# chenghuige/golden-huffman

Measured on AMD Instinct MI355X. Metric: encode+decode GB/s (input bytes), higher is better.
Workload: dtype u8

## Files before the change

### golden-huffman_amd/csrc/ghf_api.hip

```cpp
#include <algorithm>
#include <cstdio>
#include <cstring>
#include <new>
#include <string>

#include "ghf_code_rules.h"
#include "ghf_ctx.h"

using namespace ghf;

namespace {

thread_local std::string g_create_err;

int ensure_ws(ghf_ctx* c, size_t nchunks) {
  bool new_off = false, new_hist = false;
  int rc = grow(c, c->chunk_off, nchunks + 1, 1024, &new_off);
  if (!rc) rc = grow(c, c->chunk_hist, nchunks * 256, 1024 * 256, &new_hist);
  if (new_off) c->plan.forget();
  if (new_hist) c->hist.forget();
  return rc;
}

}
// ... 178 lines not shown
}

const char* ghf_last_error(ghf_ctx* c) { return c ? c->err.c_str() : g_create_err.c_str(); }

int ghf_device_alloc(ghf_ctx* c, size_t bytes, void** d_ptr) {
  if (!c || !d_ptr) return GHF_E_INVAL;
  GHF_HIP(c, hipSetDevice(c->device));
  GHF_HIP(c, hipMalloc(d_ptr, bytes ? bytes : 16));
  return GHF_OK;
}
int ghf_device_free(ghf_ctx* c, void* d_ptr) {
  if (!c) return GHF_E_INVAL;
  if (d_ptr) {
    GHF_HIP(c, hipSetDevice(c->device));
    GHF_HIP(c, hipStreamSynchronize(c->stream));
    GHF_HIP(c, hipFree(d_ptr));
  }
  return GHF_OK;
}
int ghf_host_alloc(ghf_ctx* c, size_t bytes, void** h_ptr) {
  if (!c || !h_ptr) return GHF_E_INVAL;
  GHF_HIP(c, hipSetDevice(c->device));
  GHF_HIP(c, hipHostMalloc(h_ptr, bytes ? bytes : 16, hipHostMallocDefault));
  return GHF_OK;
}
int ghf_host_free(ghf_ctx* c, void* h_ptr) {
  if (!c) return GHF_E_INVAL;
  if (h_ptr) GHF_HIP(c, hipHostFree(h_ptr));
  return GHF_OK;
}
int ghf_copy_h2d(ghf_ctx* c, void* d_dst, const void* h_src, size_t bytes) {
  if (!c || (bytes && (!d_dst || !h_src))) return GHF_E_INVAL;
  GHF_HIP(c, hipSetDevice(c->device));
  if (bytes) GHF_HIP(c, hipMemcpyAsync(d_dst, h_src, bytes, hipMemcpyHostToDevice, c->stream));
  return GHF_OK;
}
int ghf_copy_d2h(ghf_ctx* c, void* h_dst, const void* d_src, size_t bytes) {
  if (!c || (bytes && (!h_dst || !d_src))) return GHF_E_INVAL;
  GHF_HIP(c, hipSetDevice(c->device));
  if (bytes) GHF_HIP(c, hipMemcpyAsync(h_dst, d_src, bytes, hipMemcpyDeviceToHost, c->stream));
  return GHF_OK;
}
int ghf_copy_d2d(ghf_ctx* c, void* d_dst, const void* d_src, size_t bytes, int non_temporal) {
  if (!c || (bytes && (!d_dst || !d_src))) return GHF_E_INVAL;
  if (!aligned16(d_dst) || !aligned16(d_src)) return fail(c, GHF_E_INVAL, "ghf_copy_d2d: 16-byte aligned pointers");
  GHF_HIP(c, hipSetDevice(c->device));
  if (bytes) launch_stream_copy(static_cast<const uint8_t*>(d_src), static_cast<uint8_t*>(d_dst), bytes, non_temporal != 0, c->stream);
  return GHF_OK;
}
int ghf_memset_d(ghf_ctx* c, void* d_dst, int value, size_t bytes) {
  if (!c || (bytes && !d_dst)) return GHF_E_INVAL;
  GHF_HIP(c, hipSetDevice(c->device));
  if (bytes) GHF_HIP(c, hipMemsetAsync(d_dst, value, bytes, c->stream));
  return GHF_OK;
}

struct ghf_event {
  int device = 0;
  hipEvent_t ev = nullptr;
};
int ghf_event_create(ghf_ctx* c, ghf_event** out) {
  if (!c || !out) return GHF_E_INVAL;
  GHF_HIP(c, hipSetDevice(c->device));
  ghf_event* e = new (std::nothrow) ghf_event;
  if (!e) return fail(c, GHF_E_HIP, "out of host memory");
  e->device = c->device;
  const hipError_t rc = hipEventCreateWithFlags(&e->ev, hipEventDisableTiming);
  if (rc != hipSuccess) {
    delete e;
    return fail(c, GHF_E_HIP, "hipEventCreateWithFlags", rc);
  }
  *out = e;
  return GHF_OK;
}
int ghf_event_destroy(ghf_event* e) {
  if (!e) return GHF_OK;
  (void)hipSetDevice(e->device);
  if (e->ev) (void)hipEventDestroy(e->ev);
  delete e;
  return GHF_OK;
}
int ghf_event_record(ghf_ctx* c, ghf_event* e) {
  if (!c || !e) return GHF_E_INVAL;
  GHF_HIP(c, hipSetDevice(c->device));
  GHF_HIP(c, hipEventRecord(e->ev, c->stream));
  return GHF_OK;
}
int ghf_event_wait(ghf_ctx* c, ghf_event* e) {
  if (!c || !e) return GHF_E_INVAL;
  GHF_HIP(c, hipSetDevice(c->device));
  GHF_HIP(c, hipStreamWaitEvent(c->stream, e->ev, 0));
  return GHF_OK;
}
int ghf_event_sync(ghf_event* e) {
  if (!e) return GHF_E_INVAL;
  if (hipSetDevice(e->device) != hipSuccess) return GHF_E_HIP;
  return hipEventSynchronize(e->ev) == hipSuccess ? GHF_OK : GHF_E_HIP;
}

uint32_t ghf_chunk_symbols(size_t n) { return chunk_symbols_for(n); }
size_t ghf_header_bytes(int max_len) { return header_bytes_for((size_t)max_len); }

size_t ghf_compress_bound(size_t n) {
  const size_t bits = 9 * (n + 1);
  size_t b = header_bytes_for(32) + (bits + 7) / 8;
  return ((b + 15) & ~(size_t)15) + 16;
}

static int histogram(ghf_ctx* c, const uint8_t* d_in, size_t n, uint64_t* d_hist, bool add) {
  if (!c || !d_hist || (n && !d_in)) return GHF_E_INVAL;
  GHF_HIP(c, hipSetDevice(c->device));
  const uint32_t cl = chunk_symbols_for(n);
  const size_t nchunks = (size_t)chunk_count_for(n);
  int rc = ensure_ws(c, nchunks);
  if (rc) return rc;
  launch_histogram(d_in, n, cl, (uint32_t)nchunks, c->chunk_hist.p, d_hist, c->d_hist_acc, add, c->stream);
  GHF_HIP(c, hipGetLastError());
  if (add) c->hist.forget();
  else c->hist = {d_in, n, cl};
  return GHF_OK;
}
int ghf_histogram(ghf_ctx* c, const uint8_t* d_in, size_t n, uint64_t* d_hist) { return histogram(c, d_in, n, d_hist, false); }
int ghf_histogram_add(ghf_ctx* c, const uint8_t* d_in, size_t n, uint64_t* d_hist) { return histogram(c, d_in, n, d_hist, true); }

int ghf_build_code_ex(ghf_ctx* c, const uint64_t* d_hist, ghf_code* d_code, unsigned flags) {
  if (!c || !d_hist || !d_code || (flags & ~(unsigned)(GHF_CODE_LIMIT | GHF_EMPTY_OK))) return GHF_E_INVAL;
  GHF_HIP(c, hipSetDevice(c->device));
  launch_build_code(d_hist, d_code, c->d_status, flags, c->stream);
  GHF_HIP(c, hipGetLastError());
  if (c->plan.code == d_code) c->plan.forget();
  if (c->prepared.describes(d_code)) c->prepared.forget();
  return GHF_OK;
}

int ghf_build_code(ghf_ctx* c, const uint64_t* d_hist, ghf_code* d_code) { return ghf_build_code_ex(c, d_hist, d_code, 0); }

int ghf_write_header(ghf_ctx* c, const ghf_code* d_code, uint8_t* d_out, size_t cap) {
  if (!c || !d_code || !d_out || (reinterpret_cast<uintptr_t>(d_out) & 3u)) return GHF_E_INVAL;
  GHF_HIP(c, hipSetDevice(c->device));
  launch_write_header(d_code, d_out, cap, c->d_status, c->stream);
  GHF_HIP(c, hipGetLastError());
  return GHF_OK;
}

int ghf_encode_plan(ghf_ctx* c, const uint8_t* d_in, size_t n, const ghf_code* d_code, uint64_t* d_total_bits) {
  if (!c || !d_code || (n && !d_in)) return GHF_E_INVAL;
  GHF_HIP(c, hipSetDevice(c->device));
  const uint32_t cl = chunk_symbols_for(n);
  const size_t nchunks = (size_t)chunk_count_for(n);
  int rc = ensure_ws(c, nchunks);
  if (rc) return rc;
  const bool have_hist = c->hist.describes(d_in, n, cl) && n != 0;
  launch_plan(d_in, n, cl, (uint32_t)nchunks, have_hist ? c->chunk_hist.p : nullptr, d_code, c->chunk_off.p,
              d_total_bits ? d_total_bits : &c->d->total_bits, c->stream);
  GHF_HIP(c, hipGetLastError());
  c->plan = {d_in, n, d_code};
  return GHF_OK;
}

int ghf_encode_emit(ghf_ctx* c, const uint8_t* d_in, size_t n, const ghf_code* d_code, const uint64_t* d_start_bit,
                    int flags, uint8_t* d_out, size_t cap, const ghf_index* index, uint64_t* d_end) {
  if (!c || !d_code || !d_out || (n && !d_in)) return GHF_E_INVAL;
  if (!aligned16(d_out)) return fail(c, GHF_E_INVAL, "d_out must be 16-byte aligned");
  if ((flags & GHF_EMIT_HEADER) && (flags & GHF_EMIT_REBASE))
    return fail(c, GHF_E_INVAL, "GHF_EMIT_HEADER is for the buffer that starts at stream byte 0 (rank 0 / single GPU)");
  if (!c->plan.describes(d_in, n, d_code))
    return fail(c, GHF_E_INVAL, "ghf_encode_emit: call ghf_encode_plan on the same (d_in, n, d_code) first");
  GHF_HIP(c, hipSetDevice(c->device));
  const uint32_t cl = chunk_symbols_for(n);
  const size_t nchunks = (size_t)chunk_count_for(n);
  if (index && (index->n_symbols != n || !index_has_arrays(index)))
    return fail(c, GHF_E_INVAL, "ghf_encode_emit: index does not match n (use ghf_index_alloc)");
  EmitParams p;
  p.in = d_in;
  p.n = n;
  p.code = d_code;
  p.chunk_off = c->chunk_off.p;
  p.d_start_bit = d_start_bit;
  p.out = d_out;
  p.cap = cap;
  p.chunk = cl;
  p.nchunks = (uint32_t)nchunks;
  p.chunk_bit = index ? index->d_chunk_bit : nullptr;
  p.seg_bit = index ? index->d_seg_bit : nullptr;
  p.flags = flags;
  p.status = c->d_status;
  p.d_end = d_end;
  launch_emit(p, c->stream);
  GHF_HIP(c, hipGetLastError());
  return GHF_OK;
}

int ghf_shard_start_bit(ghf_ctx* c, const ghf_code* d_code, const uint64_t* d_totals, int world, int rank,
                        uint64_t* d_start_bit) {
  if (!c || !d_code || !d_totals || !d_start_bit || world < 1 || rank < 0 || rank >= world) return GHF_E_INVAL;
  GHF_HIP(c, hipSetDevice(c->device));
  launch_shard_start(d_code, d_totals, rank, d_start_bit, c->stream);
  GHF_HIP(c, hipGetLastError());
  return GHF_OK;
}

int ghf_compress(ghf_ctx* c, const uint8_t* d_in, size_t n, uint8_t* d_out, size_t cap, uint64_t* d_out_bytes,
                 ghf_code* d_code, const ghf_index* index) {
  return ghf_compress_ex(c, d_in, n, d_out, cap, d_out_bytes, d_code, index, 0);
}

int ghf_compress_ex(ghf_ctx* c, const uint8_t* d_in, size_t n, uint8_t* d_out, size_t cap, uint64_t* d_out_bytes,
                    ghf_code* d_code, const ghf_index* index, unsigned code_flags) {
  if (!c || !d_out || (n && !d_in)) return GHF_E_INVAL;
  if (n == 0 && !(code_flags & GHF_EMPTY_OK)) return fail(c, GHF_E_EMPTY, "empty input is undefined in the reference; refused");
  if (!aligned16(d_out)) return fail(c, GHF_E_INVAL, "d_out must be 16-byte aligned");
  ghf_code* code = d_code ? d_code : c->d_code;
  int rc;
  if (n == 0) {
    const size_t hdr = ghf_header_bytes(1);
    if (cap < hdr + 1) return fail(c, GHF_E_CAP, "ghf_compress: capacity below the 1049 bytes of the empty stream");
    if ((rc = ghf_histogram(c, d_in, 0, c->d_hist))) return rc;
    if ((rc = ghf_build_code_ex(c, c->d_hist, code, code_flags))) return rc;
    if ((rc = ghf_write_header(c, code, d_out, cap))) return rc;
    GHF_HIP(c, hipMemsetAsync(d_out + hdr, 0x7F, 1, c->stream));
    if (d_out_bytes) {
      launch_store_u64(d_out_bytes, nullptr, hdr + 1, c->stream);
      GHF_HIP(c, hipGetLastError());
    }
    return GHF_OK;
  }
  if ((rc = ghf_histogram(c, d_in, n, c->d_hist))) return rc;
  if ((rc = ghf_build_code_ex(c, c->d_hist, code, code_flags))) return rc;
  if ((rc = ghf_encode_plan(c, d_in, n, code, &c->d->total_bits))) return rc;
  if ((rc = ghf_encode_emit(c, d_in, n, code, nullptr, GHF_EMIT_LAST | GHF_EMIT_HEADER, d_out, cap, index, c->d->end))) return rc;
  if (d_out_bytes) {
    launch_store_u64(d_out_bytes, &c->d->end[1], 0, c->stream);
    GHF_HIP(c, hipGetLastError());
  }
  return GHF_OK;
}

int ghf_index_alloc(ghf_ctx* c, size_t n_symbols, ghf_index* out) {
  if (!c || !out) return GHF_E_INVAL;
  GHF_HIP(c, hipSetDevice(c->device));
  std::memset(out, 0, sizeof *out);
  index_shape(n_symbols, out);
  GHF_HIP(c, hipMalloc(&out->d_chunk_bit, std::max<size_t>(out->n_chunks, 1) * sizeof(uint64_t)));
  hipError_t e = hipMalloc(&out->d_seg_bit, std::max<size_t>(out->n_segs, 1) * sizeof(uint32_t));
  if (e != hipSuccess) {
    (void)hipFree(out->d_chunk_bit);
    out->d_chunk_bit = nullptr;
    return fail(c, GHF_E_HIP, "hipMalloc(seg_bit)", e);
  }
  return GHF_OK;
}

int ghf_index_free(ghf_ctx* c, ghf_index* idx) { return free_index_arrays(c, idx); }

size_t ghf_compress_batch_bound(size_t max_item_bytes) { return ghf_compress_bound(max_item_bytes); }

int ghf_batch_index_alloc(ghf_ctx* c, uint32_t count, size_t max_item_bytes, ghf_batch_index* out) {
  if (!c || !out || max_item_bytes == 0 || max_item_bytes > GHF_BATCH_MAX_ITEM) return GHF_E_INVAL;
  GHF_HIP(c, hipSetDevice(c->device));
  std::memset(out, 0, sizeof *out);
  out->count = count;
  out->max_item_bytes = max_item_bytes;
  out->blocks_per_item = blocks_for(max_item_bytes);
  out->segs_per_item = segs_for(max_item_bytes);
  GHF_HIP(c, hipMalloc(&out->d_chunk_bit, std::max<size_t>((size_t)count * out->blocks_per_item, 1) * sizeof(uint64_t)));
  hipError_t e = hipMalloc(&out->d_seg_bit, std::max<size_t>((size_t)count * out->segs_per_item, 1) * sizeof(uint32_t));
  if (e != hipSuccess) {
    (void)hipFree(out->d_chunk_bit);
    out->d_chunk_bit = nullptr;
    return fail(c, GHF_E_HIP, "hipMalloc(batch seg_bit)", e);
  }
  return GHF_OK;
}

int ghf_batch_index_free(ghf_ctx* c, ghf_batch_index* idx) { return free_index_arrays(c, idx); }

int ghf_batch_index_item(const ghf_batch_index* idx, uint32_t i, size_t n_i, ghf_index* view) {
  if (!idx || !view || i >= idx->count || n_i > idx->max_item_bytes) return GHF_E_INVAL;
  std::memset(view, 0, sizeof *view);
  index_shape(n_i, view);
  view->d_chunk_bit = idx->d_chunk_bit ? idx->d_chunk_bit + (size_t)i * idx->blocks_per_item : nullptr;
  view->d_seg_bit = idx->d_seg_bit ? idx->d_seg_bit + (size_t)i * idx->segs_per_item : nullptr;
  return GHF_OK;
}

static bool batch_index_covers(const ghf_batch_index* ix, uint32_t count, size_t max_item_bytes) {
  return ix->d_chunk_bit && ix->d_seg_bit && ix->count >= count && ix->max_item_bytes >= max_item_bytes &&
         ix->max_item_bytes <= GHF_BATCH_MAX_ITEM &&
         ix->blocks_per_item == blocks_for(ix->max_item_bytes) && ix->segs_per_item == segs_for(ix->max_item_bytes);
}

int ghf_compress_batch(ghf_ctx* c, const uint8_t* const* d_in_ptrs, const uint64_t* d_in_bytes, size_t max_item_bytes,
                       uint32_t count, uint8_t* const* d_out_ptrs, const uint64_t* d_out_caps, uint64_t* d_out_bytes,
                       ghf_code* d_codes, const ghf_batch_index* index, int* d_item_status) {
  if (!c) return GHF_E_INVAL;
  if (max_item_bytes == 0 || max_item_bytes > GHF_BATCH_MAX_ITEM)
    return fail(c, GHF_E_INVAL, "ghf_compress_batch: max_item_bytes must be 1 .. GHF_BATCH_MAX_ITEM");
  if (index && !batch_index_covers(index, count, max_item_bytes))
    return fail(c, GHF_E_INVAL, "ghf_compress_batch: index does not cover (count, max_item_bytes) (use ghf_batch_index_alloc)");
  if (count == 0) return GHF_OK;
  if (!d_in_ptrs || !d_in_bytes || !d_out_ptrs || !d_out_caps || !d_out_bytes || !d_item_status) return GHF_E_INVAL;
  GHF_HIP(c, hipSetDevice(c->device));
  if (!d_codes) {
    const int rc = grow(c, c->batch_codes, count);
    if (rc) return rc;
    d_codes = c->batch_codes.p;
  }
// ... 1095 lines not shown
```

### golden-huffman_amd/csrc/ghf_internal.h

```cpp
#ifndef GHF_INTERNAL_H_
#define GHF_INTERNAL_H_
#include <hip/hip_runtime.h>
#include <stdint.h>
#include <type_traits>
#include "ghf.h"

namespace ghf {

constexpr int kWave = 64;
constexpr int kSymPerLane = 16;
constexpr int kSymPerIter = kWave * kSymPerLane;
constexpr int kSegSymbols = 64;
constexpr int kBlockSymbols = 4096;
constexpr uint32_t kChunkQuantum = 4096;
constexpr uint32_t kMinChunk = 16384;
constexpr uint32_t kMaxChunk = 1u << 20;
constexpr uint32_t kEmitSlots = 256 * 3 * 8;

constexpr int kHistThreads = 256;
constexpr int kHistRep = 32;

constexpr int kEmitThreads = 512;
constexpr int kEmitWaves = kEmitThreads / kWave;
constexpr int kStageWords = 544;
// ... 191 lines not shown
};

struct BatchHistParams {
  const uint8_t* const* in_ptrs;
  const uint64_t* in_bytes;
  uint64_t max_item_bytes;
  uint32_t count;
  uint64_t* hist;
};
struct BatchSharedCompressParams {
  const uint8_t* const* in_ptrs;
  const uint64_t* in_bytes;
  uint64_t max_item_bytes;
  const ghf_code* code;
  uint8_t* const* out_ptrs;
  const uint64_t* out_caps;
  uint64_t* out_bytes;
  uint64_t* chunk_bit;
  uint32_t* seg_bit;
  uint64_t blocks_per_item, segs_per_item;
  int* item_status;
};
struct BatchSharedDecodeParams {
  const uint8_t* const* stream_ptrs;
  const uint64_t* stream_bytes;
  const ghf_code* code;
  const uint64_t* chunk_bit;
  const uint32_t* seg_bit;
  uint64_t blocks_per_item, segs_per_item;
  uint64_t max_item_bytes;
  const uint64_t* n_symbols;
  uint8_t* const* out_ptrs;
  const uint64_t* out_caps;
  uint64_t* out_bytes;
  int* item_status;
};
struct BatchSharedBodiesParams {
  const uint8_t* const* stream_ptrs;
  const uint64_t* stream_bytes;
  uint64_t max_stream_bytes;
  const ghf_code* code;
  uint8_t* const* out_ptrs;
  const uint64_t* out_caps;
  uint64_t* out_bytes;
  int* item_status;
  uint64_t* stats;
};

struct BatchPlanesHistParams {
  const uint8_t* const* in_ptrs;
  const uint64_t* in_bytes;
  uint64_t max_item_bytes;
  uint32_t count;
  uint64_t* hists;
};
struct BatchPlanesCompressParams {
  const uint8_t* const* in_ptrs;
  const uint64_t* in_bytes;
  uint64_t max_item_bytes;
  const ghf_code* codes;
  uint8_t* const* out_ptrs;
  const uint64_t* out_caps;
  uint64_t* out_bytes;
  uint64_t* chunk_bit;
  uint32_t* seg_bit;
  uint64_t blocks_per_item, segs_per_item;
  int* item_status;
};
struct BatchPlanesDecodeParams {
  const uint8_t* const* stream_ptrs;
  const uint64_t* stream_bytes;
  const ghf_code* codes;
  const uint64_t* chunk_bit;
  const uint32_t* seg_bit;
  uint64_t blocks_per_item, segs_per_item;
  uint64_t max_plane_symbols;
  const uint64_t* n_elems;
  uint8_t* const* out_ptrs;
  const uint64_t* out_caps;
  uint64_t* out_bytes;
  int* item_status;
};
struct BatchPlanesBodiesParams {
  const uint8_t* const* stream_ptrs;
  const uint64_t* stream_bytes;
  uint64_t max_stream_bytes;
  const ghf_code* codes;
  uint8_t* const* out_ptrs;
  const uint64_t* out_caps;
  uint64_t* out_bytes;
  int* item_status;
  uint64_t* stats;
};

constexpr uint32_t kBatchSeekMagic = 0x31524247u;
constexpr uint32_t kBatchRunSymbols = 128;
constexpr uint32_t kBatchRunSegs = kBatchRunSymbols / kSegSymbols;
constexpr uint32_t kBatchRunsPerBlock = kBlockSymbols / kBatchRunSymbols;
constexpr uint32_t kBatchSeekHeadBytes = 8;
__host__ __device__ constexpr inline uint64_t batch_runs_for(uint64_t n) { return (n + kBatchRunSymbols - 1) / kBatchRunSymbols; }
__host__ __device__ constexpr inline uint64_t batch_seek_bytes_for(uint64_t n) {
  return (kBatchSeekHeadBytes + 2 * batch_runs_for(n) + 7) & ~7ull;
}
struct BatchSeekPackParams {
  const uint64_t* chunk_bit;
  const uint32_t* seg_bit;
  uint64_t blocks_per_item, segs_per_item;
  uint64_t max_slice_symbols;
  const uint64_t* in_bytes;
  uint32_t elem_bytes;
  uint8_t* const* rec_ptrs;
  const uint64_t* rec_caps;
  uint64_t* rec_bytes;
  int* slot_status;
};
struct BatchSeekDecodeParams {
  const uint8_t* const* stream_ptrs;
  const uint64_t* stream_bytes;
  const uint8_t* const* rec_ptrs;
  const uint64_t* rec_bytes;
  uint64_t max_stream_bytes;
  const ghf_code* codes;
  uint8_t* const* out_ptrs;
  const uint64_t* out_caps;
  uint64_t* out_bytes;
  int* item_status;
};

enum SyncKind : uint32_t {
  kSyncCrs2 = 0,
  kSyncCrs = 1,
  kSyncPiece = 2,
};
struct SyncParams {
  const uint8_t* stream;
  uint64_t stream_bytes;
  uint64_t body_bit0;
  uint64_t end_bit;
  uint32_t no_eof;
  const DecTables* dt;
  uint64_t nsub;
  uint16_t* start;
  uint16_t* used;
  uint32_t* cnt;
  uint8_t* eof;
  uint32_t first;
  uint32_t first_start;
  uint32_t* changed;
  unsigned long long* moved_first_inv;
  uint64_t* eof_sub;
  uint64_t* tile_sum;
};

constexpr size_t kHistAccWords = 32 * 256 + 16 + 16 * 16;
void launch_histogram(const uint8_t* d_in, uint64_t n, uint32_t chunk, uint32_t nchunks, uint32_t* d_chunk_hist,
                      uint64_t* d_hist, uint64_t* d_acc, bool add, hipStream_t s);
void launch_build_code(const uint64_t* d_hist, ghf_code* d_code, int* d_status, uint32_t flags, hipStream_t s);
void launch_write_header(const ghf_code* d_code, uint8_t* d_out, uint64_t cap, int* d_status, hipStream_t s);
void launch_plan(const uint8_t* d_in, uint64_t n, uint32_t chunk, uint32_t nchunks, const uint32_t* d_chunk_hist,
                 const ghf_code* d_code, uint64_t* d_chunk_off, uint64_t* d_total_bits, hipStream_t s);
void launch_scan(uint64_t* d_v, uint32_t count, uint64_t* d_total, hipStream_t s);
void launch_crs_build_code(const uint64_t* d_hist, ghf_tree* d_tree, ghf_code* d_code, uint64_t* d_start_bit, int* d_status,
                           hipStream_t s);
void launch_crs_finish(const ghf_tree* d_tree, const uint64_t* d_total_bits, uint8_t* d_out, uint64_t* d_out_bytes, int* d_status,
                       hipStream_t s);
void launch_stream_copy(const uint8_t* d_src, uint8_t* d_dst, uint64_t n, bool nt, hipStream_t s);
void launch_store_u64(uint64_t* d_dst, const uint64_t* d_src_opt, uint64_t add, hipStream_t s);
void launch_load_u16(uint64_t* d_dst, const uint16_t* d_src, hipStream_t s);
void launch_shard_start(const ghf_code* d_code, const uint64_t* d_totals, int rank, uint64_t* d_start_bit, hipStream_t s);
void launch_emit(const EmitParams& p, hipStream_t s);
void launch_build_decode_tables(const ghf_code* d_code, DecTables* d_dt, int* d_status, hipStream_t s);
void launch_build_decode_tables_slots(const ghf_code* d_codes, DecTables* d_dts, uint32_t count, uint32_t slots, int* d_status, hipStream_t s);
void launch_crs_decode_tables(const ghf_tree* d_tree, DecTables* d_dt, int* d_status, hipStream_t s);
constexpr uint64_t kDecMaxGroups = 0xFFFF0000ull;
void launch_decode(const DecParams& p, hipStream_t s);
void launch_sync_pass(const SyncParams& p, hipStream_t s);
void launch_sync_counts(const SyncParams& p, uint64_t* d_total, hipStream_t s);
size_t sync_scan_workspace(uint64_t nsub);
void launch_sync_scan(const SyncParams& p, uint8_t* ws, uint32_t stride ,
                      uint32_t entry , hipStream_t s);
void launch_sync_index(const SyncParams& p, uint64_t* d_seg_abs, uint64_t n_symbols, uint64_t* d_chunk_bit, uint32_t* d_seg_bit,
                       hipStream_t s);
void launch_seek_pack(const SeekPackParams& p, hipStream_t s);
void launch_seek_expand(const SeekExpandParams& p, hipStream_t s);
void launch_seek_expand_planes(const SeekExpandPlanesParams& a, uint32_t planes, hipStream_t s);
void launch_seek_expand_streams(const SeekExpandStreamsParams& a, uint32_t streams, hipStream_t s);
void launch_decode_head(const DecHeadParams& p, hipStream_t s);
void launch_compress_batch(const BatchCompressParams& p, uint32_t count, hipStream_t s);
void launch_decode_batch(const BatchDecodeParams& p, uint32_t count, hipStream_t s);
void launch_decode_images_batch(const BatchImagesParams& p, uint32_t count, hipStream_t s);
void launch_histogram_batch(const BatchHistParams& p, uint32_t flags, hipStream_t s);
void launch_compress_batch_shared(const BatchSharedCompressParams& p, uint32_t count, hipStream_t s);
void launch_decode_batch_shared(const BatchSharedDecodeParams& p, uint32_t count, hipStream_t s);
void launch_decode_bodies_batch_shared(const BatchSharedBodiesParams& p, uint32_t count, hipStream_t s);
void launch_histogram_batch_finish(uint64_t* d_hists, uint32_t n_hists, uint32_t flags, hipStream_t s);
void launch_histogram_batch_planes(const BatchPlanesHistParams& p, uint32_t elem_bytes, uint32_t flags, hipStream_t s);
void launch_build_codes(const uint64_t* d_hists, uint32_t n_codes, ghf_code* d_codes, int* d_status, uint32_t flags, hipStream_t s);
void launch_batch_planes_raw_auto(const uint64_t* d_hists, const ghf_code* d_codes, uint32_t elem_bytes, uint32_t* d_raw_planes,
                                  hipStream_t s);
void launch_compress_batch_planes(const BatchPlanesCompressParams& p, uint32_t count, uint32_t elem_bytes, bool forms, uint32_t raw_planes,
                                  hipStream_t s);
void launch_decode_batch_planes(const BatchPlanesDecodeParams& p, uint32_t count, uint32_t elem_bytes, bool forms, uint32_t raw_planes,
                                hipStream_t s);
void launch_decode_bodies_batch_planes(const BatchPlanesBodiesParams& p, uint32_t count, uint32_t elem_bytes, bool forms,
                                       uint32_t raw_planes, hipStream_t s);
void launch_batch_seek_pack(const BatchSeekPackParams& p, uint32_t slots, hipStream_t s);
void launch_decode_bodies_batch_seek(const BatchSeekDecodeParams& p, uint32_t count, uint32_t elem_bytes, bool forms, uint32_t raw_planes,
                                     hipStream_t s);
void launch_planes_split(const uint8_t* d_in, const uint8_t* d_base, uint64_t n_elems, uint32_t elem_bytes, uint8_t* d_planes,
                         uint64_t plane_stride, hipStream_t s);
void launch_planes_merge(const uint8_t* d_planes, uint64_t plane_stride, const uint8_t* d_base, uint64_t n_elems, uint32_t elem_bytes,
                         uint8_t* d_out, const int* d_status, hipStream_t s);
void launch_planes_merge_range(const uint8_t* d_planes, uint64_t plane_stride, const uint8_t* d_base, uint64_t first, uint64_t count,
                               uint32_t elem_bytes, uint8_t* d_out, const int* d_status, hipStream_t s);
void launch_planes_split_to(const uint8_t* d_in, const uint8_t* d_base, uint64_t n_elems, uint32_t elem_bytes, uint8_t* const* h_dst,
                            hipStream_t s);
void launch_planes_merge_from(const uint8_t* const* h_src, const uint8_t* d_base, uint64_t n_elems, uint32_t elem_bytes, uint8_t* d_out,
                              const int* d_status, hipStream_t s);
void launch_sparse_split(const uint8_t* d_in, uint64_t n, uint8_t* d_mask, uint8_t* d_vals, uint64_t vals_cap, uint64_t* d_n_vals,
                         uint64_t* d_counts, uint64_t* d_offs, int* d_status, hipStream_t s);
void launch_sparse_merge(const uint8_t* d_mask, const uint8_t* d_vals, uint64_t n_vals, uint64_t n, uint8_t* d_out, uint64_t* d_counts,
                         uint64_t* d_offs, int* d_status, hipStream_t s);
void launch_sparse_merge_at(const uint8_t* d_mask, const uint8_t* d_vals, uint64_t vals_skip, uint64_t n_vals, uint64_t n, uint8_t* d_out,
                            uint64_t* d_counts, uint64_t* d_offs, int* d_status, hipStream_t s);
void launch_sparse_rank_pack(const uint8_t* d_mask, uint64_t n, uint8_t* d_table, uint64_t* d_counts, uint64_t* d_offs, int* d_status,
                             hipStream_t s);
hipError_t launch_histogram_planes(const uint8_t* d_in, const uint8_t* d_base, uint64_t n_elems, uint32_t elem_bytes, uint32_t flags,
                                   uint64_t* d_acc, uint64_t* d_hists, hipStream_t s);
void launch_planes_image_bytes(const uint64_t* d_hists, const ghf_code* d_codes, uint32_t elem_bytes, uint64_t* d_bytes, hipStream_t s);
void launch_planes_vet_codes(const uint64_t* d_hists, const ghf_code* d_codes, uint32_t elem_bytes, int* d_status, hipStream_t s);

struct PlanesGatherParams {
  const uint8_t* streams[GHF_PLANES_MAX];
  uint64_t stream_bytes[GHF_PLANES_MAX];
  const uint8_t* records[GHF_PLANES_MAX];
  const ghf_code* codes;
  uint64_t n_elems, n_blocks;
  const uint64_t* index;
  uint64_t index_stride;
  uint32_t row_elems, n_rows;
  uint32_t stage_bytes;
  uint8_t* out;
  uint64_t out_stride;
  int32_t* row_status;
};
void launch_decode_planes_gather(const PlanesGatherParams& p, uint32_t elem_bytes, uint32_t raw_planes, hipStream_t s);

}
#endif
```

### golden-huffman_amd/csrc/ghf_kernels.hip

```cpp
#include "ghf_build_code.h"

namespace ghf {

#define GHF_HADD(x, sh) atomicAdd(&lh[((((x) >> (sh)) & 0xFFu) << 5) | rep], 1u)

__device__ __forceinline__ void hist_vec(uint32_t* lh, uint32_t rep, const uint4& v) {
  GHF_HADD(v.x, 0); GHF_HADD(v.x, 8); GHF_HADD(v.x, 16); GHF_HADD(v.x, 24);
  GHF_HADD(v.y, 0); GHF_HADD(v.y, 8); GHF_HADD(v.y, 16); GHF_HADD(v.y, 24);
  GHF_HADD(v.z, 0); GHF_HADD(v.z, 8); GHF_HADD(v.z, 16); GHF_HADD(v.z, 24);
  GHF_HADD(v.w, 0); GHF_HADD(v.w, 8); GHF_HADD(v.w, 16); GHF_HADD(v.w, 24);
}

__global__ __launch_bounds__(kHistThreads) void k_histogram(const uint8_t* __restrict__ in, uint64_t n,
                                                            uint32_t chunk32, uint32_t nchunks,
                                                            uint32_t* __restrict__ chunk_hist,
                                                            unsigned long long* __restrict__ hist,
                                                            unsigned long long* __restrict__ acc ,
                                                            uint32_t add ) {
  static_assert(kHistRep == 32, "replica index is lane % 32");
  __shared__ uint32_t lh[256 * kHistRep];
  __shared__ bool s_last;
  const uint32_t tid = threadIdx.x;
  const uint32_t rep = tid & 31u;
  uint32_t prev = 0;
// ... 194 lines not shown
  for (int s = lane; s < GHF_NSYM; s += 64) heap.cur[s] = (uint16_t)s;
  for (int i = lane; i < GHF_NSYM + 256 + 7; i += 64) {
    heap.parent[i] = 0;
    T.size[i] = 1;
    T.is_right[i] = 0;
  }
  for (int i = lane; i < (int)(sizeof(ghf_tree) / 4); i += 64) reinterpret_cast<uint32_t*>(&tree)[i] = 0;
  if (lane == 0) {
    T.max_len = 0;
    T.min_len = 0xFFFFFFFFu;
  }
  __syncthreads();
  int n = 0;
  for (int s = 0; s < 256; ++s) {
    const u64t f = wave_uniform((u64t)hist[s]);
    if (f) {
      wave_heap_push(heap, n, (f << 9) | (u64t)s, lane);
      ++n;
    }
  }
  const int nleaves = n;
  if (nleaves < 2) {
    if (lane == 0) latch_status(status, nleaves == 0 ? GHF_E_EMPTY : GHF_E_SINGLE);
    return;
  }
  const int times = n - 1;
  for (int t = 0; t < times; ++t) {
    const u64t e1 = wave_heap_pop(heap, n, lane);
    const u64t e2 = wave_heap_pop(heap, n, lane);
    const int s1 = (int)(e1 & 511u), s2 = (int)(e2 & 511u);
    const int node = GHF_NSYM + t;
    if (lane == 0) {
      const int a = heap.cur[s1], b = heap.cur[s2];
      heap.parent[a] = (uint16_t)node;
      heap.parent[b] = (uint16_t)node;
      T.tl[t] = (uint16_t)a;
      T.tr[t] = (uint16_t)b;
      T.is_right[b] = 1;
      T.size[node] = (uint16_t)(1 + T.size[a] + T.size[b]);
      heap.cur[s2] = (uint16_t)node;
    }
    wave_heap_push(heap, n, (((e1 >> 9) + (e2 >> 9)) << 9) | (u64t)s2, lane);
    ++n;
  }
  __syncthreads();
  for (int v = lane; v < GHF_NSYM + times; v += 64) {
    const bool leaf = v < 256;
    if (v == 256 || (leaf && heap.parent[v] == 0)) continue;
    uint32_t len = 0, pre = 0;
    unsigned long long code = 0;
    int x = v;
    for (int p; (p = heap.parent[x]) != 0; x = p) {
      const uint32_t r = T.is_right[x];
      if (len < 64) code |= (unsigned long long)r << len;
      ++len;
      pre += 1u + (r ? (uint32_t)T.size[T.tl[p - GHF_NSYM]] : 0u);
    }
    if (leaf) {
      tree.header[2 * pre] = 0;
      tree.header[2 * pre + 1] = (uint8_t)v;
      atomicMax(&T.max_len, len);
      atomicMin(&T.min_len, len);
      if (len <= 64) {
        out_code->length[v] = len;
        out_code->codeword[v] = (uint32_t)code;
        T.code_hi[v] = (uint32_t)(code >> 32);
      }
    } else {
      tree.header[2 * pre] = 255;
      tree.header[2 * pre + 1] = 255;
      const int t = v - GHF_NSYM;
      const int a = T.tl[t], b = T.tr[t];
      tree.left[t] = (uint16_t)(a < GHF_NSYM ? a : 256 + (a - GHF_NSYM));
      tree.right[t] = (uint16_t)(b < GHF_NSYM ? b : 256 + (b - GHF_NSYM));
    }
  }
  __syncthreads();
  const bool deep = T.max_len > 32u;
  for (int s = lane; s < GHF_NSYM; s += 64) {
    const bool absent = s == 256 || heap.parent[s] == 0;
    if (absent) {
      out_code->length[s] = 0;
      out_code->codeword[s] = 0;
    }
    out_code->symbol[s] = deep ? (absent ? 0u : T.code_hi[s]) : 0xFFFFFFFFu;
  }
  for (int i = lane; i < 64; i += 64) {
    out_code->first_code[i] = 0;
    out_code->start_pos[i] = 0;
  }
  if (T.max_len > 64u) {
    if (lane == 0) latch_status(status, GHF_E_CODELEN);
    return;
  }
  if (lane == 0) {
    tree.root = (uint32_t)(256 + times - 1);
    tree.n_leaves = (uint32_t)nleaves;
    tree.max_len = T.max_len;
    tree.tree_bytes = 2u * (2u * (uint32_t)nleaves - 1u);
    out_code->min_len = (int32_t)T.min_len;
    out_code->max_len = (int32_t)T.max_len;
    if (start_bit) *start_bit = 8ull * ((unsigned long long)tree.tree_bytes + 2ull);
  }
  __syncthreads();
  for (int i = lane; i < (int)(sizeof(ghf_tree) / 4); i += 64)
    reinterpret_cast<uint32_t*>(out_tree)[i] = reinterpret_cast<const uint32_t*>(&tree)[i];
}

void launch_crs_build_code(const uint64_t* d_hist, ghf_tree* d_tree, ghf_code* d_code, uint64_t* d_start_bit, int* d_status,
                           hipStream_t s) {
  hipLaunchKernelGGL(k_crs_build_code, dim3(1), dim3(64), 0, s, reinterpret_cast<const unsigned long long*>(d_hist), d_tree,
                     d_code, reinterpret_cast<unsigned long long*>(d_start_bit), d_status);
}

__global__ __launch_bounds__(256) void k_crs_finish(const ghf_tree* __restrict__ tree, const unsigned long long* __restrict__ total_bits,
                                                    uint8_t* __restrict__ out, unsigned long long* __restrict__ out_bytes,
                                                    const int* __restrict__ status) {
  if (*status != 0) return;
  const uint32_t tb = tree->tree_bytes;
  for (uint32_t i = threadIdx.x; i < tb; i += 256) out[i] = tree->header[i];
  if (threadIdx.x == 0) {
    const unsigned long long t = *total_bits;
    const unsigned long long whole = t >> 3;
    const uint32_t left = (uint32_t)((8u - (uint32_t)(t & 7u)) & 7u);
    out[tb] = (uint8_t)left;
    out[tb + 1] = left ? out[tb + 2 + whole] : (uint8_t)0;
    if (out_bytes) *out_bytes = (unsigned long long)tb + 2ull + whole;
  }
}

void launch_crs_finish(const ghf_tree* d_tree, const uint64_t* d_total_bits, uint8_t* d_out, uint64_t* d_out_bytes, int* d_status,
                       hipStream_t s) {
  hipLaunchKernelGGL(k_crs_finish, dim3(1), dim3(256), 0, s, d_tree, reinterpret_cast<const unsigned long long*>(d_total_bits), d_out,
                     reinterpret_cast<unsigned long long*>(d_out_bytes), d_status);
}

__global__ __launch_bounds__(256) void k_write_header(const ghf_code* __restrict__ code, uint8_t* __restrict__ out,
                                                      uint64_t cap, int* __restrict__ status) {
  const int max_len = code->max_len;
  if (max_len < 1 || max_len > 32) return;
  const int nwords = 1 + GHF_NSYM + 2 + 2 * max_len;
  if ((uint64_t)nwords * 4 > cap) {
    if (threadIdx.x == 0) latch_status(status, GHF_E_CAP);
    return;
  }
  uint32_t* o = reinterpret_cast<uint32_t*>(out);
  for (int w = threadIdx.x; w < nwords; w += blockDim.x) o[w] = bswap32(header_word(code, w, max_len));
}

void launch_write_header(const ghf_code* d_code, uint8_t* d_out, uint64_t cap, int* d_status, hipStream_t s) {
  hipLaunchKernelGGL(k_write_header, dim3(1), dim3(256), 0, s, d_code, d_out, cap, d_status);
}

__global__ __launch_bounds__(256) void k_chunk_bits(const uint32_t* __restrict__ chunk_hist, uint32_t nchunks,
                                                    const ghf_code* __restrict__ code, uint64_t* __restrict__ bits) {
  const int lane = threadIdx.x & 63;
  const uint32_t wave = (blockIdx.x * blockDim.x + threadIdx.x) >> 6;
  const uint32_t nwaves = (gridDim.x * blockDim.x) >> 6;
  const uint4 L = reinterpret_cast<const uint4*>(code->length)[lane];
  for (uint32_t c = wave; c < nchunks; c += nwaves) {
    const uint4 h = reinterpret_cast<const uint4*>(chunk_hist + (uint64_t)c * 256)[lane];
    unsigned long long b = (unsigned long long)h.x * L.x + (unsigned long long)h.y * L.y +
                           (unsigned long long)h.z * L.z + (unsigned long long)h.w * L.w;
#pragma unroll
    for (int d = 32; d >= 1; d >>= 1) b += __shfl_xor(b, d, 64);
    if (lane == 0) bits[c] = b;
  }
}

__global__ __launch_bounds__(256) void k_chunk_bits_direct(const uint8_t* __restrict__ in, uint64_t n, uint32_t chunk32,
                                                           uint32_t nchunks, const ghf_code* __restrict__ code,
                                                           uint64_t* __restrict__ bits) {
  __shared__ uint32_t ll[256];
  ll[threadIdx.x] = code->length[threadIdx.x];
  __syncthreads();
  const int lane = threadIdx.x & 63;
  const uint32_t wave = (blockIdx.x * blockDim.x + threadIdx.x) >> 6;
  const uint32_t nwaves = (gridDim.x * blockDim.x) >> 6;
  const uint64_t chunk = chunk32;
  for (uint32_t c = wave; c < nchunks; c += nwaves) {
    const uint64_t base = (uint64_t)c * chunk;
    const uint64_t len = (n - base < chunk) ? (n - base) : chunk;
    unsigned long long b = 0;
    const uint8_t* p = in + base;
    uint64_t head = (16u - (uint32_t)((uintptr_t)p & 15u)) & 15u;
    if (head > len) head = len;
    if ((uint64_t)lane < head) b += ll[p[lane]];
    const uint4* pv = reinterpret_cast<const uint4*>(p + head);
    const uint64_t nvec = (len - head) >> 4;
    uint32_t acc = 0;
    for (uint64_t i = lane; i < nvec; i += 64) {
      const uint4 v = pv[i];
      const uint32_t w[4] = {v.x, v.y, v.z, v.w};
#pragma unroll
      for (int k = 0; k < 4; ++k)
        acc += ll[w[k] & 0xFFu] + ll[(w[k] >> 8) & 0xFFu] + ll[(w[k] >> 16) & 0xFFu] + ll[w[k] >> 24];
      if ((i >> 6) % 4096u == 4095u) {
        b += acc;
        acc = 0;
      }
    }
    b += acc;
    const uint64_t tail0 = head + (nvec << 4);
    if (tail0 + (uint64_t)lane < len) b += ll[p[tail0 + lane]];
#pragma unroll
    for (int d = 32; d >= 1; d >>= 1) b += __shfl_xor(b, d, 64);
    if (lane == 0) bits[c] = b;
  }
}

__global__ __launch_bounds__(1024) void k_scan(uint64_t* __restrict__ v, uint32_t count, uint64_t* __restrict__ total_out) {
  __shared__ unsigned long long wsum[16];
  const int tid = threadIdx.x, lane = tid & 63, w = tid >> 6;
  const uint32_t ipt = (count + 1023u) / 1024u;
  const uint32_t lo = tid * ipt;
  const uint32_t hi = (lo + ipt < count) ? lo + ipt : count;
  unsigned long long mine = 0;
  const bool small = ipt <= 8u;
  unsigned long long x8[8];
  if (small) {
#pragma unroll
    for (uint32_t k = 0; k < 8; ++k) {
      const uint32_t i = lo + k;
      x8[k] = (k < ipt && i < hi) ? v[i] : 0ull;
    }
#pragma unroll
    for (uint32_t k = 0; k < 8; ++k) mine += x8[k];
  } else {
    for (uint32_t i = lo; i < hi; ++i) mine += v[i];
  }
  unsigned long long s = mine;
#pragma unroll
  for (int d = 1; d < 64; d <<= 1) {
    const unsigned long long t = __shfl_up(s, d, 64);
    if (lane >= d) s += t;
  }
  if (lane == 63) wsum[w] = s;
  __syncthreads();
  unsigned long long woff = 0, total = 0;
  for (int k = 0; k < 16; ++k) {
    const unsigned long long x = wsum[k];
    if (k < w) woff += x;
    total += x;
  }
  unsigned long long run = woff + s - mine;
  if (small) {
#pragma unroll
    for (uint32_t k = 0; k < 8; ++k) {
      const uint32_t i = lo + k;
      if (k < ipt && i < hi) v[i] = run;
      run += x8[k];
    }
  } else {
    for (uint32_t i = lo; i < hi; ++i) {
      const unsigned long long x = v[i];
      v[i] = run;
      run += x;
    }
  }
  if (tid == 0) {
    v[count] = total;
    if (total_out) *total_out = total;
  }
}

void launch_scan(uint64_t* d_v, uint32_t count, uint64_t* d_total, hipStream_t s) {
  hipLaunchKernelGGL(k_scan, dim3(1), dim3(1024), 0, s, d_v, count, d_total);
}

void launch_plan(const uint8_t* d_in, uint64_t n, uint32_t chunk, uint32_t nchunks, const uint32_t* d_chunk_hist,
                 const ghf_code* d_code, uint64_t* d_chunk_off, uint64_t* d_total_bits, hipStream_t s) {
  uint32_t blocks = (nchunks + 3) / 4;
  if (blocks > 2048) blocks = 2048;
  if (blocks == 0) blocks = 1;
  if (d_chunk_hist)
    hipLaunchKernelGGL(k_chunk_bits, dim3(blocks), dim3(256), 0, s, d_chunk_hist, nchunks, d_code, d_chunk_off);
  else
    hipLaunchKernelGGL(k_chunk_bits_direct, dim3(blocks), dim3(256), 0, s, d_in, n, chunk, nchunks, d_code,
                       d_chunk_off);
  hipLaunchKernelGGL(k_scan, dim3(1), dim3(1024), 0, s, d_chunk_off, nchunks, d_total_bits);
}

__global__ void k_store_u64(uint64_t* dst, const uint64_t* src, uint64_t add) { *dst = (src ? *src : 0ull) + add; }
void launch_store_u64(uint64_t* d_dst, const uint64_t* d_src_opt, uint64_t add, hipStream_t s) {
  hipLaunchKernelGGL(k_store_u64, dim3(1), dim3(1), 0, s, d_dst, d_src_opt, add);
}

__global__ void k_load_u16(uint64_t* dst, const uint16_t* src) { *dst = *src; }
void launch_load_u16(uint64_t* d_dst, const uint16_t* d_src, hipStream_t s) { hipLaunchKernelGGL(k_load_u16, dim3(1), dim3(1), 0, s, d_dst, d_src); }

__global__ void k_shard_start(const ghf_code* code, const uint64_t* totals, int rank, uint64_t* start_bit) {
  uint64_t b = 8ull * header_bytes_for((uint64_t)code->max_len);
  for (int r = 0; r < rank; ++r) b += totals[r];
  *start_bit = b;
}
void launch_shard_start(const ghf_code* d_code, const uint64_t* d_totals, int rank, uint64_t* d_start_bit, hipStream_t s) {
  hipLaunchKernelGGL(k_shard_start, dim3(1), dim3(1), 0, s, d_code, d_totals, rank, d_start_bit);
}

template <bool NT>
__global__ __launch_bounds__(256) void k_stream_copy(const uint4* __restrict__ src, uint4* __restrict__ dst, uint64_t nvec) {
  const uint64_t per = (nvec + gridDim.x - 1) / gridDim.x;
  const uint64_t lo = (uint64_t)blockIdx.x * per;
  const uint64_t end = lo + per < nvec ? lo + per : nvec;
  uint64_t i = lo + threadIdx.x;
  auto ld = [&](uint64_t k) -> uint4 { return NT ? load_stream(src + k) : src[k]; };
  auto st = [&](uint64_t k, const uint4& v) {
    if (NT) store_stream(dst + k, v);
    else dst[k] = v;
  };
  for (; i + 3 * 256 < end; i += 4 * 256) {
    const uint4 a = ld(i), b = ld(i + 256), c = ld(i + 512), d = ld(i + 768);
    st(i, a); st(i + 256, b); st(i + 512, c); st(i + 768, d);
  }
  for (; i < end; i += 256) st(i, ld(i));
}
__global__ void k_tail_copy(const uint8_t* src, uint8_t* dst, uint64_t from, uint64_t n) {
  const uint64_t i = from + threadIdx.x;
  if (i < n) dst[i] = src[i];
}
void launch_stream_copy(const uint8_t* d_src, uint8_t* d_dst, uint64_t n, bool nt, hipStream_t s) {
  const uint64_t nvec = n / 16;
  if (nvec) {
    uint64_t blocks = (nvec + 255) / 256;
    if (blocks > 4096) blocks = 4096;
    if (nt) hipLaunchKernelGGL(k_stream_copy<true>, dim3((uint32_t)blocks), dim3(256), 0, s, reinterpret_cast<const uint4*>(d_src), reinterpret_cast<uint4*>(d_dst), nvec);
    else hipLaunchKernelGGL(k_stream_copy<false>, dim3((uint32_t)blocks), dim3(256), 0, s, reinterpret_cast<const uint4*>(d_src), reinterpret_cast<uint4*>(d_dst), nvec);
  }
  if (n & 15) hipLaunchKernelGGL(k_tail_copy, dim3(1), dim3(16), 0, s, d_src, d_dst, nvec * 16, n);
}

}
```

Before: 969.7.

## Fuse chunk-bit computation and offset scan into one last-block-scan plan kernel

```diff
diff --git a/golden-huffman_amd/csrc/ghf_api.hip b/golden-huffman_amd/csrc/ghf_api.hip
--- a/golden-huffman_amd/csrc/ghf_api.hip
+++ b/golden-huffman_amd/csrc/ghf_api.hip
@@ -354,7 +354,7 @@
   if (rc) return rc;
   const bool have_hist = c->hist.describes(d_in, n, cl) && n != 0;
   launch_plan(d_in, n, cl, (uint32_t)nchunks, have_hist ? c->chunk_hist.p : nullptr, d_code, c->chunk_off.p,
-              d_total_bits ? d_total_bits : &c->d->total_bits, c->stream);
+              d_total_bits ? d_total_bits : &c->d->total_bits, c->d_hist_acc + kPlanTickWord, c->stream);
   GHF_HIP(c, hipGetLastError());
   c->plan = {d_in, n, d_code};
   return GHF_OK;
diff --git a/golden-huffman_amd/csrc/ghf_internal.h b/golden-huffman_amd/csrc/ghf_internal.h
--- a/golden-huffman_amd/csrc/ghf_internal.h
+++ b/golden-huffman_amd/csrc/ghf_internal.h
@@ -367,13 +367,14 @@
   uint64_t* tile_sum;
 };
 
-constexpr size_t kHistAccWords = 32 * 256 + 16 + 16 * 16;
+constexpr size_t kPlanTickWord = 32 * 256 + 16 + 16 * 16;
+constexpr size_t kHistAccWords = kPlanTickWord + 16;
 void launch_histogram(const uint8_t* d_in, uint64_t n, uint32_t chunk, uint32_t nchunks, uint32_t* d_chunk_hist,
                       uint64_t* d_hist, uint64_t* d_acc, bool add, hipStream_t s);
 void launch_build_code(const uint64_t* d_hist, ghf_code* d_code, int* d_status, uint32_t flags, hipStream_t s);
 void launch_write_header(const ghf_code* d_code, uint8_t* d_out, uint64_t cap, int* d_status, hipStream_t s);
 void launch_plan(const uint8_t* d_in, uint64_t n, uint32_t chunk, uint32_t nchunks, const uint32_t* d_chunk_hist,
-                 const ghf_code* d_code, uint64_t* d_chunk_off, uint64_t* d_total_bits, hipStream_t s);
+                 const ghf_code* d_code, uint64_t* d_chunk_off, uint64_t* d_total_bits, uint64_t* d_tick, hipStream_t s);
 void launch_scan(uint64_t* d_v, uint32_t count, uint64_t* d_total, hipStream_t s);
 void launch_crs_build_code(const uint64_t* d_hist, ghf_tree* d_tree, ghf_code* d_code, uint64_t* d_start_bit, int* d_status,
                            hipStream_t s);
diff --git a/golden-huffman_amd/csrc/ghf_kernels.hip b/golden-huffman_amd/csrc/ghf_kernels.hip
--- a/golden-huffman_amd/csrc/ghf_kernels.hip
+++ b/golden-huffman_amd/csrc/ghf_kernels.hip
@@ -370,60 +370,141 @@
   hipLaunchKernelGGL(k_write_header, dim3(1), dim3(256), 0, s, d_code, d_out, cap, d_status);
 }
 
-__global__ __launch_bounds__(256) void k_chunk_bits(const uint32_t* __restrict__ chunk_hist, uint32_t nchunks,
-                                                    const ghf_code* __restrict__ code, uint64_t* __restrict__ bits) {
-  const int lane = threadIdx.x & 63;
-  const uint32_t wave = (blockIdx.x * blockDim.x + threadIdx.x) >> 6;
+constexpr uint32_t kPlanBlocks = 128;
+
+template <bool DIRECT>
+__global__ __launch_bounds__(256) void k_plan(const uint8_t* __restrict__ in, uint64_t n, uint32_t chunk32,
+                                              const uint32_t* __restrict__ chunk_hist, uint32_t nchunks,
+                                              const ghf_code* __restrict__ code, unsigned long long* v,
+                                              unsigned long long* total_out, unsigned long long* tick) {
+  __shared__ unsigned long long wsum[4];
+  __shared__ bool s_last;
+  const uint32_t tid = threadIdx.x;
+  const int lane = tid & 63;
+  const uint32_t wave = (blockIdx.x * blockDim.x + tid) >> 6;
   const uint32_t nwaves = (gridDim.x * blockDim.x) >> 6;
-  const uint4 L = reinterpret_cast<const uint4*>(code->length)[lane];
-  for (uint32_t c = wave; c < nchunks; c += nwaves) {
-    const uint4 h = reinterpret_cast<const uint4*>(chunk_hist + (uint64_t)c * 256)[lane];
-    unsigned long long b = (unsigned long long)h.x * L.x + (unsigned long long)h.y * L.y +
-                           (unsigned long long)h.z * L.z + (unsigned long long)h.w * L.w;
+  auto put = [&](uint32_t c, unsigned long long b) { __hip_atomic_store(&v[c], b, __ATOMIC_RELAXED, __HIP_MEMORY_SCOPE_AGENT); };
+  auto wave_sum = [](unsigned long long b) {
 #pragma unroll
     for (int d = 32; d >= 1; d >>= 1) b += __shfl_xor(b, d, 64);
-    if (lane == 0) bits[c] = b;
-  }
-}
-
-__global__ __launch_bounds__(256) void k_chunk_bits_direct(const uint8_t* __restrict__ in, uint64_t n, uint32_t chunk32,
-                                                           uint32_t nchunks, const ghf_code* __restrict__ code,
-                                                           uint64_t* __restrict__ bits) {
-  __shared__ uint32_t ll[256];
-  ll[threadIdx.x] = code->length[threadIdx.x];
-  __syncthreads();
-  const int lane = threadIdx.x & 63;
-  const uint32_t wave = (blockIdx.x * blockDim.x + threadIdx.x) >> 6;
-  const uint32_t nwaves = (gridDim.x * blockDim.x) >> 6;
-  const uint64_t chunk = chunk32;
-  for (uint32_t c = wave; c < nchunks; c += nwaves) {
-    const uint64_t base = (uint64_t)c * chunk;
-    const uint64_t len = (n - base < chunk) ? (n - base) : chunk;
-    unsigned long long b = 0;
-    const uint8_t* p = in + base;
-    uint64_t head = (16u - (uint32_t)((uintptr_t)p & 15u)) & 15u;
-    if (head > len) head = len;
-    if ((uint64_t)lane < head) b += ll[p[lane]];
-    const uint4* pv = reinterpret_cast<const uint4*>(p + head);
-    const uint64_t nvec = (len - head) >> 4;
-    uint32_t acc = 0;
-    for (uint64_t i = lane; i < nvec; i += 64) {
-      const uint4 v = pv[i];
-      const uint32_t w[4] = {v.x, v.y, v.z, v.w};
-#pragma unroll
-      for (int k = 0; k < 4; ++k)
-        acc += ll[w[k] & 0xFFu] + ll[(w[k] >> 8) & 0xFFu] + ll[(w[k] >> 16) & 0xFFu] + ll[w[k] >> 24];
-      if ((i >> 6) % 4096u == 4095u) {
-        b += acc;
-        acc = 0;
+    return b;
+  };
+  if constexpr (!DIRECT) {
+    const uint32_t sub = (uint32_t)lane >> 4, j = (uint32_t)lane & 15u;
+    uint4 L[4];
+#pragma unroll
+    for (uint32_t r = 0; r < 4; ++r) L[r] = reinterpret_cast<const uint4*>(code->length)[j + 16 * r];
+    const uint64_t ngroups = ((uint64_t)nchunks + 3) / 4;
+    for (uint64_t q0 = wave; q0 < ngroups; q0 += 4ull * nwaves) {
+      uint4 h[4][4];
+#pragma unroll
+      for (uint32_t k = 0; k < 4; ++k) {
+        const uint64_t c = 4 * (q0 + (uint64_t)k * nwaves) + sub;
+        const uint4* row = reinterpret_cast<const uint4*>(chunk_hist + (c < nchunks ? c : nchunks - 1) * 256);
+#pragma unroll
+        for (uint32_t r = 0; r < 4; ++r) h[k][r] = row[j + 16 * r];
       }
-    }
-    b += acc;
-    const uint64_t tail0 = head + (nvec << 4);
-    if (tail0 + (uint64_t)lane < len) b += ll[p[tail0 + lane]];
-#pragma unroll
-    for (int d = 32; d >= 1; d >>= 1) b += __shfl_xor(b, d, 64);
-    if (lane == 0) bits[c] = b;
+#pragma unroll
+      for (uint32_t k = 0; k < 4; ++k) {
+        const uint64_t c = 4 * (q0 + (uint64_t)k * nwaves) + sub;
+        unsigned long long b = 0;
+#pragma unroll
+        for (uint32_t r = 0; r < 4; ++r)
+          b += (unsigned long long)h[k][r].x * L[r].x + (unsigned long long)h[k][r].y * L[r].y +
+               (unsigned long long)h[k][r].z * L[r].z + (unsigned long long)h[k][r].w * L[r].w;
+#pragma unroll
+        for (int d = 8; d >= 1; d >>= 1) b += __shfl_xor(b, d, 64);
+        if (j == 0 && c < nchunks) put((uint32_t)c, b);
+      }
+    }
+  } else {
+    __shared__ uint32_t ll[256];
+    ll[tid] = code->length[tid];
+    __syncthreads();
+    const uint64_t chunk = chunk32;
+    for (uint32_t c = wave; c < nchunks; c += nwaves) {
+      const uint64_t base = (uint64_t)c * chunk;
+      const uint64_t len = (n - base < chunk) ? (n - base) : chunk;
+      unsigned long long b = 0;
+      const uint8_t* p = in + base;
+      uint64_t head = (16u - (uint32_t)((uintptr_t)p & 15u)) & 15u;
+      if (head > len) head = len;
+      if ((uint64_t)lane < head) b += ll[p[lane]];
+      const uint4* pv = reinterpret_cast<const uint4*>(p + head);
+      const uint64_t nvec = (len - head) >> 4;
+      uint32_t acc = 0;
+      for (uint64_t i = lane; i < nvec; i += 64) {
+        const uint4 x = pv[i];
+        const uint32_t w[4] = {x.x, x.y, x.z, x.w};
+#pragma unroll
+        for (int k = 0; k < 4; ++k)
+          acc += ll[w[k] & 0xFFu] + ll[(w[k] >> 8) & 0xFFu] + ll[(w[k] >> 16) & 0xFFu] + ll[w[k] >> 24];
+        if ((i >> 6) % 4096u == 4095u) {
+          b += acc;
+          acc = 0;
+        }
+      }
+      b += acc;
+      const uint64_t tail0 = head + (nvec << 4);
+      if (tail0 + (uint64_t)lane < len) b += ll[p[tail0 + lane]];
+      b = wave_sum(b);
+      if (lane == 0) put(c, b);
+    }
+  }
+
+  asm volatile("s_waitcnt vmcnt(0)" ::: "memory");
+  __syncthreads();
+  if (tid == 0) {
+    const unsigned long long t = __hip_atomic_fetch_add(tick, 1ull, __ATOMIC_RELAXED, __HIP_MEMORY_SCOPE_AGENT);
+    s_last = (t + 1 == gridDim.x);
+    if (s_last) __builtin_amdgcn_fence(__ATOMIC_ACQUIRE, "agent");
+    asm volatile("s_waitcnt vmcnt(0)" ::: "memory");
+  }
+  __syncthreads();
+  if (!s_last) return;
+
+  constexpr uint32_t kRun = 32;
+  const uint64_t count = nchunks;
+  unsigned long long carry = 0;
+  for (uint64_t t0 = 0; t0 < count; t0 += 256 * kRun) {
+    const uint64_t lo = t0 + (uint64_t)tid * kRun;
+    unsigned long long x[kRun], mine = 0;
+#pragma unroll
+    for (uint32_t k = 0; k < kRun; ++k)
+      x[k] = __hip_atomic_load(&v[lo + k < count ? lo + k : count - 1], __ATOMIC_RELAXED, __HIP_MEMORY_SCOPE_AGENT);
+#pragma unroll
+    for (uint32_t k = 0; k < kRun; ++k) {
+      if (lo + k >= count) x[k] = 0;
+      mine += x[k];
+    }
+    unsigned long long s = mine;
+#pragma unroll
+    for (int d = 1; d < 64; d <<= 1) {
+      const unsigned long long t = __shfl_up(s, d, 64);
+      if (lane >= d) s += t;
+    }
+    if (t0) __syncthreads();
+    if (lane == 63) wsum[tid >> 6] = s;
+    __syncthreads();
+    unsigned long long woff = 0, total = 0;
+#pragma unroll
+    for (uint32_t k = 0; k < 4; ++k) {
+      const unsigned long long w = wsum[k];
+      if (k < (tid >> 6)) woff += w;
+      total += w;
+    }
+    unsigned long long run = carry + woff + s - mine;
+#pragma unroll
+    for (uint32_t k = 0; k < kRun; ++k) {
+      if (lo + k < count) v[lo + k] = run;
+      run += x[k];
+    }
+    carry += total;
+  }
+  if (tid == 0) {
+    v[count] = carry;
+    if (total_out) *total_out = carry;
+    __hip_atomic_store(tick, 0ull, __ATOMIC_RELAXED, __HIP_MEMORY_SCOPE_AGENT);
   }
 }
 
@@ -487,16 +568,18 @@
 }
 
 void launch_plan(const uint8_t* d_in, uint64_t n, uint32_t chunk, uint32_t nchunks, const uint32_t* d_chunk_hist,
-                 const ghf_code* d_code, uint64_t* d_chunk_off, uint64_t* d_total_bits, hipStream_t s) {
+                 const ghf_code* d_code, uint64_t* d_chunk_off, uint64_t* d_total_bits, uint64_t* d_tick, hipStream_t s) {
   uint32_t blocks = (nchunks + 3) / 4;
-  if (blocks > 2048) blocks = 2048;
+  const uint32_t most = d_chunk_hist ? kPlanBlocks : 2048u;
+  if (blocks > most) blocks = most;
   if (blocks == 0) blocks = 1;
+  unsigned long long* v = reinterpret_cast<unsigned long long*>(d_chunk_off);
+  unsigned long long* total = reinterpret_cast<unsigned long long*>(d_total_bits);
+  unsigned long long* tick = reinterpret_cast<unsigned long long*>(d_tick);
   if (d_chunk_hist)
-    hipLaunchKernelGGL(k_chunk_bits, dim3(blocks), dim3(256), 0, s, d_chunk_hist, nchunks, d_code, d_chunk_off);
+    hipLaunchKernelGGL(k_plan<false>, dim3(blocks), dim3(256), 0, s, d_in, n, chunk, d_chunk_hist, nchunks, d_code, v, total, tick);
   else
-    hipLaunchKernelGGL(k_chunk_bits_direct, dim3(blocks), dim3(256), 0, s, d_in, n, chunk, nchunks, d_code,
-                       d_chunk_off);
-  hipLaunchKernelGGL(k_scan, dim3(1), dim3(1024), 0, s, d_chunk_off, nchunks, d_total_bits);
+    hipLaunchKernelGGL(k_plan<true>, dim3(blocks), dim3(256), 0, s, d_in, n, chunk, d_chunk_hist, nchunks, d_code, v, total, tick);
 }
 
 __global__ void k_store_u64(uint64_t* dst, const uint64_t* src, uint64_t add) { *dst = (src ? *src : 0ull) + add; }
diff --git a/scratch/plan_chain_trace.py b/scratch/plan_chain_trace.py
--- /dev/null
+++ b/scratch/plan_chain_trace.py
@@ -0,0 +1,92 @@
+#!/usr/bin/env python3
+import csv, sys
+
+rows = list(csv.DictReader(open(sys.argv[1])))
+steps = int(sys.argv[2]) if len(sys.argv) > 2 else 20
+first = int(sys.argv[3]) if len(sys.argv) > 3 else 8
+
+
+def short(n):
+    n = n.replace("void ", "").replace("ghf::", "")
+    for sep in ("<", "("):
+        n = n.split(sep)[0]
+    return n.strip()
+
+
+ev = {}
+for r in rows:
+    ev.setdefault(short(r["Kernel_Name"]), []).append((int(r["Start_Timestamp"]), int(r["End_Timestamp"]), r["Stream_Id"]))
+for v in ev.values():
+    v.sort()
+
+
+def timed(name):
+    return ev.get(name, [])[-steps:]
+
+
+hist, code, tabs, emit, dec = (timed(k) for k in ("k_histogram", "k_build_code", "k_build_decode_tables", "k_emit", "k_decode"))
+plan_names = [k for k in ("k_chunk_bits", "k_scan", "k_plan") if k in ev]
+plans = {k: timed(k) for k in plan_names}
+t0 = hist[0][0]
+us = lambda t: (t - t0) / 1e3
+
+
+def after(lst, t, stream, used):
+    for j, e in enumerate(lst):
+        if j not in used and e[2] == stream and e[0] >= t - 2000:
+            used.add(j)
+            return e
+    return None
+
+
+used = {k: set() for k in plan_names + ["tabs"]}
+print("timed region: %.3f ms" % ((dec[-1][1] - t0) / 1e6))
+hdr = ["step", "K2 end"] + ["%s start..end (dur)" % k for k in plan_names] + ["tables start..end (dur)", "K2 end -> plan end", "K2 end -> tables end", "k_emit start", "tables end -> k_emit"]
+print("| " + " | ".join(hdr) + " |")
+print("|" + "---|" * len(hdr))
+lat_plan, lat_chain = [], []
+for i in range(steps):
+    s, e, st = code[i]
+    t = e
+    cells = ["%d" % i, "%.1f" % us(e)]
+    for k in plan_names:
+        x = after(plans[k], t, st, used[k])
+        cells.append("%.1f..%.1f (%.1f)" % (us(x[0]), us(x[1]), (x[1] - x[0]) / 1e3))
+        t = x[1]
+    plan_end = t
+    x = after(tabs, t, st, used["tabs"])
+    cells.append("%.1f..%.1f (%.1f)" % (us(x[0]), us(x[1]), (x[1] - x[0]) / 1e3))
+    cells.append("%.1f" % ((plan_end - e) / 1e3))
+    cells.append("%.1f" % ((x[1] - e) / 1e3))
+    cells.append("%.1f" % us(emit[i][0]))
+    cells.append("%.1f" % ((emit[i][0] - x[1]) / 1e3))
+    lat_plan.append((plan_end - e) / 1e3)
+    lat_chain.append((x[1] - e) / 1e3)
+    if i < first:
+        print("| " + " | ".join(cells) + " |")
+print("K2 end -> plan end, us: first %d steps mean %.1f max %.1f; all %d steps mean %.1f max %.1f" % (
+    first, sum(lat_plan[:first]) / first, max(lat_plan[:first]), steps, sum(lat_plan) / steps, max(lat_plan)))
+print("K2 end -> tables end, us: first %d steps mean %.1f max %.1f; all %d steps mean %.1f max %.1f" % (
+    first, sum(lat_chain[:first]) / first, max(lat_chain[:first]), steps, sum(lat_chain) / steps, max(lat_chain)))
+for k in plan_names + ["k_build_decode_tables", "k_build_code"]:
+    d = sorted((e - s) / 1e3 for s, e, _ in timed(k))
+    print("%s in the timed region: min %.1f median %.1f max %.1f us" % (k, d[0], d[len(d) // 2], d[-1]))
+
+big = sorted(hist + emit + dec)
+busy, gaps = 0, []
+cs, ce = big[0][0], big[0][1]
+for s, e, _ in big[1:]:
+    if s <= ce:
+        ce = max(ce, e)
+    else:
+        gaps.append((ce, s - ce))
+        busy += ce - cs
+        cs, ce = s, e
+busy += ce - cs
+print("a streaming kernel was running %.3f ms; gaps: %d, total %.3f ms" % (busy / 1e6, len(gaps), sum(g for _, g in gaps) / 1e6))
+chain_ends = sorted(x[1] for x in tabs)
+for at, g in sorted(gaps, key=lambda x: -x[1])[:8]:
+    end = at + g
+    prev = [c for c in chain_ends if c <= end]
+    print("  gap of %.1f us at %.3f ms; nearest end of a table build before its end: %s us earlier" % (
+        g / 1e3, (at - t0) / 1e6, "%.1f" % ((end - prev[-1]) / 1e3) if prev else "-"))
```

Result: no change. 967.8 (median of 2 runs) (-0.2%).
